# eric-zqwang/puzzlefusion-plusplus

Hardware: AMD Instinct MI355X
Metric: denoiser DDPM-step throughput (fragment*steps/s) (higher is better)
Workload: dtype f32 (GEMMs: f16x3); 1 GPU; DDPM training iteration, BASELINE configs[1]: add_noise + rotate + frozen PointNet++/VQ encode (in the loop) + DenoiserTransformer forward (dropouts on) + MSE + full backward + [encoder of iteration i+1 issued on its own stream during iteration i] AdamW; padded_slots=not evaluated (their gradient contribution is exactly zero), puzzles_per_gpu=32, fragment_slots=20, points_per_fragment=1024, valid_fragments_per_gpu=154, weights=random init, reference architecture (57.6M denoiser + 0.6M encoder params)

## Files before the change

### include/pfpp.h

```cpp
#ifndef PFPP_H_
#define PFPP_H_

#include <stddef.h>
#include <stdint.h>

#ifdef __cplusplus
extern "C" {
#endif

#define PFPP_OK 0
#define PFPP_EINVAL (-1)
#define PFPP_EUNSUPPORTED (-2)
#define PFPP_EHIP (-3)

typedef void* pfpp_stream_t;

#define PFPP_ABI_VERSION 2
int pfpp_version(void);
const char* pfpp_build_info(void);
const char* pfpp_last_error(void);
int64_t pfpp_abi_sizeof(const char* name);
int pfpp_device_cu_count(void);
int pfpp_set_attention_mode(int mode);
int pfpp_get_attention_mode(void);
// ... 491 lines not shown
int pfpp_gemm_wd_f16(const pfpp_planes* A, int64_t lda, const pfpp_pw* w, const float* bias, const float* residual, int64_t ldr, float* out,
                     int64_t ldc, int64_t M, int64_t N, int64_t K, pfpp_stream_t stream);
#define PFPP_REBLOCK_MAX 32
typedef struct pfpp_reblock_job { pfpp_planes w; int64_t N, K, ldw; void *fhi, *flo; int32_t transposed; } pfpp_reblock_job;
int pfpp_reblock_planes(const pfpp_reblock_job* jobs, int32_t n, pfpp_stream_t stream);
int pfpp_layernorm_linear_small(const float* x, const float* mod, int64_t ld_mod, const float* gamma, const float* beta,
                                const int32_t* group_batch, int64_t group_rows, const pfpp_pw* w, const float* bias, float* out,
                                int64_t ldc, const pfpp_planes* u_planes, int64_t ldu, int64_t M, int64_t N, int64_t C, float eps,
                                pfpp_stream_t stream);

typedef struct pfpp_head_params {
  pfpp_planes w0, w2;
  const float *w4, *b0, *b2, *b4;
  pfpp_planes f0, f2;
} pfpp_head_params;
typedef struct pfpp_head_grads { float *w4, *b4, *b2, *b0; } pfpp_head_grads;
int pfpp_heads_fwd(const float* pooled, const pfpp_head_params* trans, const pfpp_head_params* rot, int64_t R, int64_t C,
                   float* a0, float* v0, float* a1, float* v1, float* out, const int32_t* slot, int64_t ldo,
                   pfpp_stream_t stream);
int pfpp_heads_bwd(const float* dout, const int32_t* slot, const pfpp_head_params* trans, const pfpp_head_params* rot, int64_t R, int64_t C,
                   const float* a0, const float* v0, const float* a1, const float* v1, float* da0, float* da1, float* dp,
                   const pfpp_head_grads* g_trans, const pfpp_head_grads* g_rot, float grad_scale, float* dx, int64_t L,
                   pfpp_stream_t stream);

int pfpp_verifier_attn_fwd(const float* qkv, float* out, float* lse, const uint8_t* key_valid, int64_t B, int64_t E, int64_t H,
                           int64_t dh, float scale, float p, uint64_t seed, uint32_t site, pfpp_stream_t stream);
int pfpp_verifier_attn_bwd(const float* qkv, const float* out, const float* dout, const float* lse, float* dqkv,
                           const uint8_t* key_valid, int64_t B, int64_t E, int64_t H, int64_t dh, float scale, float p, uint64_t seed,
                           uint32_t site, pfpp_stream_t stream);
int pfpp_verifier_attn_dropout_mask(uint8_t* keep, int64_t B, int64_t H, int64_t E, float p, uint64_t seed, uint32_t site,
                                    pfpp_stream_t stream);

int pfpp_verifier_head_bce(const float* h6, const float* w, const float* b, const float* target, const uint8_t* valid,
                           const float* dlogit_in, int64_t M, int64_t C, float neg_weight, float* logits, float* dlogit, float* dh6, float* dw, float* db, float* loss,
                           int32_t* stats, float* amax, double* workspace, pfpp_stream_t stream);
int64_t pfpp_verifier_head_bce_workspace(void);

int pfpp_verifier_gelu_dropout(const float* z, float* u, int64_t n, float p, uint64_t seed, uint32_t site, pfpp_stream_t stream);
int pfpp_verifier_gelu_dropout_bwd(const float* z, const float* du, float* dz, int64_t n, float p, uint64_t seed, uint32_t site,
                                   pfpp_stream_t stream);

int pfpp_chamfer_fwd(const float* off, const float* ctr, int64_t rep, const float* tgt, float* d_src, int32_t* i_src,
                     float* d_tgt, int32_t* i_tgt, int64_t batch, int64_t n, int64_t m, pfpp_stream_t stream);
int pfpp_chamfer_bwd(const float* off, const float* ctr, int64_t rep, const float* tgt, const int32_t* i_src, const int32_t* i_tgt,
                     float* grad, int64_t batch, int64_t n, int64_t m, float scale, const float* gscale, pfpp_stream_t stream);
int pfpp_chamfer_reduce(const float* d_src, int64_t n_src, const float* d_tgt, int64_t n_tgt, float scale, float* loss,
// ... 65 lines not shown
```

### puzzlefusion-plusplus_amd/csrc/heads.hip

```cpp
#include "pfpp_common.h"

namespace {

typedef _Float16 half8 __attribute__((ext_vector_type(8)));
typedef _Float16 half4 __attribute__((ext_vector_type(4)));
typedef float f32x16 __attribute__((ext_vector_type(16)));

constexpr int HC = 512;
constexpr int HC2 = 256;
constexpr int KP = HC + 8;
constexpr int NW = 8;

__device__ __forceinline__ float silu_f(float v) { return v / (1.0f + expf(-v)); }
__device__ __forceinline__ float silu_grad(float v) {
  const float s = 1.0f / (1.0f + expf(-v));
  return s * (1.0f + v * (1.0f - s));
}

struct HeadW {
  const _Float16 *w0h, *w0l, *w2h, *w2l;
  const half8 *f0h, *f0l, *f2h, *f2l;
  const float *w4, *b0, *b2, *b4;
  float inv_s0, inv_s2;
  int n_out, c0;
// ... 64 lines not shown
  const int S = K / 16, NG = K / 64;
  half8 bh[2][4][NT], bl[2][4][NT];
  auto fetch = [&](int g, int slot) {
#pragma unroll
    for (int j = 0; j < NT; ++j)
#pragma unroll
      for (int u = 0; u < 4; ++u) {
        const size_t blk = (size_t)(tile0 + j) * S + 4 * g + u;
        bh[slot][u][j] = fh[blk * 64 + lane];
        bl[slot][u][j] = fl[blk * 64 + lane];
      }
  };
  fetch(0, 0);
  for (int g = 0; g < NG; g += 2) {
#pragma unroll
    for (int half = 0; half < 2; ++half) {
      const int gg = g + half;
      if (gg < NG) {
        fetch(gg + 1 < NG ? gg + 1 : NG - 1, half ^ 1);
        __builtin_amdgcn_sched_barrier(0);
#pragma unroll
        for (int u = 0; u < 4; ++u) {
          const half8 a_h = ah[2 * (4 * gg + u)], a_l = al[2 * (4 * gg + u)];
#pragma unroll
          for (int j = 0; j < NT; ++j) {
            acc[j] = __builtin_amdgcn_mfma_f32_32x32x16_f16(a_l, bh[half][u][j], acc[j], 0, 0, 0);
            acc[j] = __builtin_amdgcn_mfma_f32_32x32x16_f16(a_h, bl[half][u][j], acc[j], 0, 0, 0);
            acc[j] = __builtin_amdgcn_mfma_f32_32x32x16_f16(a_h, bh[half][u][j], acc[j], 0, 0, 0);
          }
        }
        __builtin_amdgcn_sched_barrier(0);
      }
    }
  }
}

__device__ __forceinline__ void zero(f32x16& a) {
#pragma unroll
  for (int e = 0; e < 16; ++e) a[e] = 0.0f;
}

__global__ __launch_bounds__(64 * NW) void heads_fwd_kernel(HeadsFwdP p) {
  extern __shared__ __align__(16) char hd_smem[];
  _Float16* sh = reinterpret_cast<_Float16*>(hd_smem);
  _Float16* sl = sh + 32 * KP;
  const int tid = threadIdx.x, lane = tid & 63, wave = tid >> 6, l31 = lane & 31, lhi = lane >> 5;
// ... 48 lines not shown
#pragma unroll
    for (int e = 0; e < 16; ++e) {
      const int row = (e & 3) + 8 * (e >> 2) + 4 * lhi;
      const float a = acc[0][e] * w.inv_s2 + b;
      const float v = silu_f(a);
      if (p.a1 && r0 + row < R) {
        p.a1[((size_t)hd * R + r0 + row) * HC2 + col] = a;
        p.v1[((size_t)hd * R + r0 + row) * HC2 + col] = v;
      }
      sv[row * (HC2 + 1) + col] = v;
    }
    __syncthreads();
    if (tid < 32 * 4) {
      const int row = tid >> 2, c = tid & 3;
      if (c < w.n_out && r0 + row < R) {
        const float* wr = w.w4 + (size_t)c * HC2;
        float s = 0.0f;
#pragma unroll 8
        for (int k = 0; k < HC2; ++k) s = fmaf(sv[row * (HC2 + 1) + k], wr[k], s);
        const int64_t orow = p.slot ? p.slot[r0 + row] : (r0 + row);
        p.out[orow * p.ldo + w.c0 + c] = s + w.b4[c];
      }
    }
  }
}

struct HeadsBwdP {
  const float* dout;
  const int32_t* slot;
  HeadW w[2];
  const float *a0, *v0, *a1, *v1;
  float *da0, *da1;
  float* dp;
  float *gw4[2], *gb4[2], *gb2[2], *gb0[2];
  float G;
  int R;
};

__device__ __forceinline__ half4 lds_rd_tr(uint32_t addr) {
  half4 v;
  asm volatile("ds_read_b64_tr_b16 %0, %1" : "=v"(v) : "v"(addr) : "memory");
  return v;
}

__device__ __forceinline__ void contract_kmajor(const _Float16* sh, const _Float16* sl, const _Float16* __restrict__ wh,
                                                const _Float16* __restrict__ wl, int K, int ldw, int n0, _Float16* patch,
// ... 137 lines not shown
        sl[row * KP + col] = l;
      }
      cs += __shfl_xor(cs, 32);
      if (lhi == 0) unsafeAtomicAdd(p.gb0[hd] + col, cs);
    }
    __syncthreads();
  }
  {
    f32x16 acc[2];
    zero(acc[0]); zero(acc[1]);
    contract_kmajor(sh, sl, w.w0h, w.w0l, HC, HC, 64 * wave, patch, acc);
#pragma unroll
    for (int j = 0; j < 2; ++j) {
      const int col = 64 * wave + 32 * j + l31;
#pragma unroll
      for (int e = 0; e < 16; ++e) {
        const int row = (e & 3) + 8 * (e >> 2) + 4 * lhi;
        if (r0 + row < R) p.dp[((size_t)hd * R + r0 + row) * HC + col] = acc[j][e] * (invG * w.inv_s0);
      }
    }
  }
}

__global__ __launch_bounds__(256) void pool_bwd2_kernel(const float* __restrict__ dp0, const float* __restrict__ dp1, float* __restrict__ dx,
                                                        int64_t n, int L, int C) {
  const int64_t i4 = ((int64_t)blockIdx.x * 256 + threadIdx.x) * 4;
  if (i4 >= n * L * C) return;
  const int64_t row = i4 / C;
  const int c = (int)(i4 - row * C);
  const int64_t f = row / L;
  const float4 a = *reinterpret_cast<const float4*>(dp0 + f * C + c);
  const float4 b = *reinterpret_cast<const float4*>(dp1 + f * C + c);
  const float inv = 1.0f / (float)L;
  float4 v;
  v.x = (a.x + b.x) * inv; v.y = (a.y + b.y) * inv; v.z = (a.z + b.z) * inv; v.w = (a.w + b.w) * inv;
  *reinterpret_cast<float4*>(dx + i4) = v;
}

bool fill_head(HeadW& w, const pfpp_head_params& h, int n_out, int c0) {
  if (!(h.w0.hi && h.w0.lo && h.w2.hi && h.w2.lo && h.w4 && h.b0 && h.b2 && h.b4)) return false;
  w.w0h = (const _Float16*)h.w0.hi; w.w0l = (const _Float16*)h.w0.lo;
  w.w2h = (const _Float16*)h.w2.hi; w.w2l = (const _Float16*)h.w2.lo;
  const bool frag = h.f0.hi && h.f0.lo && h.f2.hi && h.f2.lo;
  w.f0h = frag ? (const half8*)h.f0.hi : nullptr; w.f0l = frag ? (const half8*)h.f0.lo : nullptr;
  w.f2h = frag ? (const half8*)h.f2.hi : nullptr; w.f2l = frag ? (const half8*)h.f2.lo : nullptr;
  w.w4 = h.w4; w.b0 = h.b0; w.b2 = h.b2; w.b4 = h.b4;
  w.inv_s0 = 1.0f / h.w0.scale; w.inv_s2 = 1.0f / h.w2.scale;
  w.n_out = n_out; w.c0 = c0;
  return true;
}

}

extern "C" int pfpp_heads_fwd(const float* pooled, const pfpp_head_params* trans, const pfpp_head_params* rot, int64_t R, int64_t C,
                              float* a0, float* v0, float* a1, float* v1, float* out, const int32_t* slot, int64_t ldo,
                              pfpp_stream_t stream) {
  PFPP_REQUIRE(pooled && trans && rot && out, "null pointer");
  PFPP_SUPPORTED(C == HC, "width != 512");
  PFPP_REQUIRE((!a0 && !v0 && !a1 && !v1) || (a0 && v0 && a1 && v1), "the saved activations come all or none");
  PFPP_REQUIRE(ldo >= 7 && pfpp::aligned16(pooled), "ldo < 7 or misaligned input");
  if (R == 0) return PFPP_OK;
  HeadsFwdP p;
  PFPP_REQUIRE(fill_head(p.w[0], *trans, 3, 0) && fill_head(p.w[1], *rot, 4, 3), "null weight pointer");
  p.x = pooled; p.a0 = a0; p.v0 = v0; p.a1 = a1; p.v1 = v1; p.out = out; p.slot = slot; p.ldo = (int)ldo; p.R = (int)R;
  const size_t smem = (size_t)2 * 32 * KP * sizeof(_Float16);
  if (pfpp_allow_dyn_lds<heads_fwd_kernel>((int)smem) != hipSuccess) return pfpp::check_launch(__func__);
  hipLaunchKernelGGL(heads_fwd_kernel, dim3((unsigned)((R + 31) / 32), 2), dim3(64 * NW), smem, pfpp::as_stream(stream), p);
  return pfpp::check_launch(__func__);
}

extern "C" int pfpp_heads_bwd(const float* dout, const int32_t* slot, const pfpp_head_params* trans, const pfpp_head_params* rot, int64_t R, int64_t C,
                              const float* a0, const float* v0, const float* a1, const float* v1, float* da0, float* da1, float* dp,
                              const pfpp_head_grads* g_trans, const pfpp_head_grads* g_rot, float grad_scale, float* dx, int64_t L,
                              pfpp_stream_t stream) {
  PFPP_REQUIRE(dout && trans && rot && a0 && v0 && a1 && v1 && da0 && da1 && dp && g_trans && g_rot, "null pointer");
  PFPP_SUPPORTED(C == HC, "width != 512");
  PFPP_REQUIRE(grad_scale > 0.0f && L >= 1, "bad grad_scale / L");
  if (R == 0) return PFPP_OK;
  HeadsBwdP p;
  PFPP_REQUIRE(fill_head(p.w[0], *trans, 3, 0) && fill_head(p.w[1], *rot, 4, 3), "null weight pointer");
  const pfpp_head_grads* gs[2] = {g_trans, g_rot};
  for (int h = 0; h < 2; ++h) {
    PFPP_REQUIRE(gs[h]->w4 && gs[h]->b4 && gs[h]->b2 && gs[h]->b0, "null gradient pointer");
    p.gw4[h] = gs[h]->w4; p.gb4[h] = gs[h]->b4; p.gb2[h] = gs[h]->b2; p.gb0[h] = gs[h]->b0;
  }
  p.dout = dout; p.slot = slot; p.a0 = a0; p.v0 = v0; p.a1 = a1; p.v1 = v1; p.da0 = da0; p.da1 = da1; p.dp = dp; p.G = grad_scale; p.R = (int)R;
  hipStream_t st = pfpp::as_stream(stream);
  const size_t smem = (size_t)2 * 32 * KP * sizeof(_Float16) + (size_t)NW * 8192;
  if (pfpp_allow_dyn_lds<heads_bwd_kernel>((int)smem) != hipSuccess) return pfpp::check_launch(__func__);
  hipLaunchKernelGGL(heads_bwd_kernel, dim3((unsigned)((R + 31) / 32), 2), dim3(64 * NW), smem, st, p);
  if (dx) {
    const int64_t total = R * L * C;
    hipLaunchKernelGGL(pool_bwd2_kernel, dim3((unsigned)((total / 4 + 255) / 256)), dim3(256), 0, st, dp, dp + R * C, dx, R, (int)L, (int)C);
  }
  return pfpp::check_launch(__func__);
}
```

### puzzlefusion-plusplus_amd/pfpp_hip/_lib.py

```python
from __future__ import annotations

import ctypes as C
import os
from pathlib import Path

LIB_PATH = Path(os.environ["PFPP_LIB_PATH"]).resolve() if os.environ.get("PFPP_LIB_PATH") else Path(__file__).resolve().parent / "libpfpp_hip.so"

_p = C.c_void_p
_i64 = C.c_int64
_i32 = C.c_int32
_f32 = C.c_float


class GemmArgs(C.Structure):

    _fields_ = [
        ("A", _p), ("W", _p), ("C", _p),
        ("w_hi", _p), ("w_lo", _p),
        ("a_hi", _p), ("a_lo", _p), ("c_hi", _p), ("c_lo", _p),
        ("bias", _p), ("scale", _p), ("shift", _p), ("residual", _p),
        ("M", _i64), ("N", _i64), ("K", _i64),
        ("lda", _i64), ("ldw", _i64), ("ldc", _i64), ("ldr", _i64),
        ("w_kmajor", _i32), ("act", _i32), ("pool", _i32),
        ("batch", _i32), ("zdiv", _i32), ("precision", _i32),
# ... 141 lines not shown

class DwJob(C.Structure):

    _fields_ = [("dy", PlanesC), ("x", PlanesC), ("gw", _p), ("gb", _p), ("M", _i64), ("N", _i64)]


class ReblockJob(C.Structure):

    _fields_ = [("w", PlanesC), ("N", _i64), ("K", _i64), ("ldw", _i64), ("fhi", _p), ("flo", _p), ("transposed", _i32)]


SIGNATURES = {
    "pfpp_tlayers_eval": [C.POINTER(TlayersEvalArgs), _p],
    "pfpp_embed_tokens_small": [_p, _p, _p, _p, _p, C.POINTER(PwC), _p, _p, _p, _p, _p, _p, _i64, _i64, _i64, _p],
    "pfpp_gemm_small": [_pl, _i64, C.POINTER(PwC), _p, _p, _i64, _p, _i64, _i64, _i64, _i64, _p],
    "pfpp_gemm_wd": [_pl, _i64, C.POINTER(PwC), _p, _p, _i64, _p, _i64, _i64, _i64, _i64, _p],
    "pfpp_gemm_wd_supported": [_i64, _i64, _i64],
    "pfpp_gemm_wd_f16": [_pl, _i64, C.POINTER(PwC), _p, _p, _i64, _p, _i64, _i64, _i64, _i64, _p],
    "pfpp_reblock_planes": [C.POINTER(ReblockJob), _i32, _p],
    "pfpp_layernorm_linear_small": [_p, _p, _i64, _p, _p, _p, _i64, C.POINTER(PwC), _p, _p, _i64, _pl, _i64, _i64, _i64, _i64, _f32, _p],
    "pfpp_heads_fwd": [_p, C.POINTER(HeadParams), C.POINTER(HeadParams), _i64, _i64, _p, _p, _p, _p, _p, _p, _i64, _p],
    "pfpp_heads_bwd": [_p, _p, C.POINTER(HeadParams), C.POINTER(HeadParams), _i64, _i64, _p, _p, _p, _p, _p, _p, _p,
                       C.POINTER(HeadGrads), C.POINTER(HeadGrads), _f32, _p, _i64, _p],
    "pfpp_tlayers_fwd": [C.POINTER(TlayersArgs), _i32, _i32, _p],
    "pfpp_tlayers_bwd": [C.POINTER(TlayersArgs), _i32, _i32, _p, _p],
    "pfpp_set_attention_mode": [C.c_int],
    "pfpp_se3_rotate_gather": [_p, _p, _p, _p, _i64, _i64, _p],
    "pfpp_pose_apply": [_p, _p, _p, _p, _i64, _i64, C.c_int, _p],
    "pfpp_fps": [_p, _p, _p, _i64, _i64, _i64, _p],
    "pfpp_ball_query": [_p, _p, _p, _i64, _i64, _i64, _i64, _f32, _p],
    "pfpp_sample_levels": [_p, _i64, _i64, C.POINTER(SampleLevel), _p],
    "pfpp_group_gather": [_p, _p, _p, _p, _p, _i64, _i64, _i64, _i64, _i64, _i64, _p],
    "pfpp_gemm": [C.POINTER(GemmArgs), _p],
    "pfpp_sa_mlp3_fused": [_p] * 16 + [_i64] * 7 + [_p],
    "pfpp_sa_mlp2_fused": [_p] * 13 + [_i64] * 7 + [_p],
    "pfpp_sa_mlp2_fused_p": [_p] * 13 + [_pl] + [_i64] * 7 + [_p],
    "pfpp_sa_mlp2_table_p": [_p] * 11 + [_pl] + [_i64] * 8 + [_p],
    "pfpp_sa_table_planes": [_p] * 7 + [_pl] + [_i64] * 6 + [_p],
    "pfpp_vq_encode": [_p, _p, _p, _p, _p, _i64, _i64, _i64, _i64, _p],
    "pfpp_scatter_rows": [_p, _p, _p, _i64, _i64, _p],
    "pfpp_token_features": [_p, _p, _p, _p, _p, _p, _i64, _i64, _p],
    "pfpp_token_features_slots": [_p, _p, _p, _p, _p, _p, _p, _i64, _i64, _p],
    "pfpp_token_combine_slots": [_p, _p, _p, _p, _p, _p, _p, _p, _i64, _i64, _i64, _p],
    "pfpp_token_combine_bwd_slots": [_p, _p, _p, _p, _p, _i64, _i64, _i64, _p],
    "pfpp_mse_loss_masked": [_p, _p, _p, _p, _p, _p, _p, _i64, _i64, _f32, _p],
    "pfpp_token_combine": [_p, _p, _p, _p, _p, _p, _i64, _i64, _i64, _i64, _p],
# ... 89 lines not shown
    "pfpp_mesh_status": [_p, _p],
    "pfpp_match_classify_compact": [_p, _p, _p, _p, _f32, _p, _p, _i64, _i64, _p, _p, _p, _p, _p],
    "pfpp_match_gather_rows": [_p, _p, _p, _p, _p, _p, _p, _i64, _i64, _i64, _p, _p, _p],
    "pfpp_match_normalize_halves": [_p, _i64, _i64, _p],
    "pfpp_sinkhorn_masked": [_p, _i64, _p, _i64, _f32, _i64, _p, _p, _p, _p, _i64, _p],
    "pfpp_fracture_labels": [_p, _p, _p, _p, _i64, _i64, _p, _p, _p],
    "pfpp_ragged_fps": [_p, _p, _p, _i64, _i64, _i64, _p, _p, _p],
    "pfpp_ragged_knn": [_p, _p, _p, _p, _i64, _i64, _i64, _i64, _p, _p, _p],
    "pfpp_ragged_group": [_p, _i64, _i64, _p, _p, _p, _i64, _i64, _i64, _i64, _p, _i64, _p],
    "pfpp_ragged_interp": [_p, _p, _p, _p, _p, _i64, _p, _i64, _i64, _i64, _p, _i64, _p, _p],
    "pfpp_feat_knn": [_p, _i64, _p, _i64, _i64, _i64, _i64, _i64, _p, _p],
    "pfpp_ptf_aggregate": [_p, _p, _p, _i64, _p, _p, _p, _p, _i64, _i64, _i64, _p, _p],
    "pfpp_attn_rows16": [_p, _p, _p, _p, _i64, _i64, _i64, _i64, _f32, _p],
    "pfpp_layernorm128": [_p, _p, _p, _p, _i64, _i64, _f32, _p],
}
PLAIN = {
    "pfpp_version": ([], C.c_int),
    "pfpp_last_error": ([], C.c_char_p),
    "pfpp_build_info": ([], C.c_char_p),
    "pfpp_abi_sizeof": ([C.c_char_p], C.c_int64),
    "pfpp_last_gemm_kernel": ([], C.c_char_p),
    "pfpp_device_cu_count": ([], C.c_int),
    "pfpp_get_attention_mode": ([], C.c_int),
    "pfpp_ada_linear_bwd_scratch_floats": ([_i64, _i64], C.c_int64),
    "pfpp_token_features_t_cols": ([_i64, _i64], C.c_int64),
    "pfpp_tlayers_fwd_bytes": ([_i64, _i64, _i64, _i64], C.c_int64),
    "pfpp_tlayers_frag_bytes": ([_i64, _i64], C.c_int64),
    "pfpp_tlayers_fwd_hout_offset": ([_i64, _i64, _i64, _i64], C.c_int64),
    "pfpp_tlayers_bwd_bytes": ([_i64, _i64, _i64, _i64], C.c_int64),
    "pfpp_bn_stats_workspace": ([_i64, _i64], C.c_int64),
    "pfpp_fragment_prepare_workspace": ([_i64, _i64], C.c_int64),
    "pfpp_verifier_head_bce_workspace": ([], C.c_int64),
    "pfpp_vq_train_workspace": ([_i64, _i64], C.c_int64),
    "pfpp_bn_relu_bwd_workspace": ([_i64, _i64], C.c_int64),
    "pfpp_mesh_vertex_graph_workspace": ([_p, _i64, _p], C.c_int64),
    "pfpp_sinkhorn_workspace": ([_i64], C.c_int64),
}

STRUCT_MIRRORS = {
    "sample_level": SampleLevel, "gemm_args": GemmArgs, "planes": PlanesC, "slab_job": SlabJob, "gemm_planes_args": GemmPlanesArgs,
    "sa_train_args": SaTrainArgs, "gemm_grad_args": GemmGradArgs, "tlayer_params": TlayerParams, "tlayer_grads": TlayerGrads,
    "tlayer_adamw": TlayerAdamw, "tlayers_args": TlayersArgs, "pw": PwC, "elayer_params": ElayerParams,
    "tlayers_eval_args": TlayersEvalArgs, "head_params": HeadParams, "head_grads": HeadGrads, "reblock_job": ReblockJob, "dw_job": DwJob,
}

ACT = {"none": 0, "relu": 1, "silu": 2, "gelu": 3, "geglu": 4}
# ... 75 lines not shown
```

### puzzlefusion-plusplus_amd/pfpp_hip/train_ops.py

```python
from __future__ import annotations

import ctypes as C
from typing import Optional, Tuple

import torch

from . import _lib
from ._lib import ACT, GemmGradArgs, check
from . import ops
from .ops import _chk, _ptr, _stream

_f32 = torch.float32
import os as _os

SPLIT_DX = _os.environ.get("PFPP_SPLIT_DX", "1") == "1"


def gemm_grad(A: torch.Tensor, W: torch.Tensor, out: torch.Tensor, *, M: int, N: int, K: int, lda: int, ldw: int,
              ldc: int, a_kmajor: bool = False, w_kmajor: bool = False, accumulate: bool = False,
              split_k: int = 0, batch: int = 1, sA: int = 0, sW: int = 0, sC: int = 0, a_scale: float = 1.0,
              w_scale: float = 1.0, alpha: float = 1.0, a_off: int = 0, w_off: int = 0, c_off: int = 0,
              colsum: Optional[torch.Tensor] = None) -> torch.Tensor:
    _chk(A, _f32, "A"); _chk(W, _f32, "W"); _chk(out, _f32, "out")
    a = GemmGradArgs()
# ... 617 lines not shown
def attn_blockdiag_bwd_planes(qkv, dout, n_frag: int, L: int, H: int, dh: int, scale: float, g_scale: float):
    from .planes import Planes, _pl

    _chk(qkv, _f32, "qkv"); _chk(dout, _f32, "dout")
    dq = Planes.empty(qkv.shape[0], qkv.shape[1], qkv.device, g_scale)
    check(_lib.load().pfpp_attn_blockdiag_bwd_p(_ptr(qkv), _ptr(dout), None, n_frag, L, H, dh, scale, _pl(dq), _stream()),
          "pfpp_attn_blockdiag_bwd_p")
    return dq


def head_params(w0, w2, w4: torch.Tensor, b0: torch.Tensor, b2: torch.Tensor, b4: torch.Tensor, static: bool = False):
    from ._lib import HeadParams, PlanesC

    for t_, nm in ((w4, "w4"), (b0, "b0"), (b2, "b2"), (b4, "b4")):
        _chk(t_, _f32, nm)
    f0 = f2 = PlanesC(None, None, 0.0)
    if static:
        (h0, l0), (h2, l2) = w0.frag(), w2.frag()
        f0, f2 = PlanesC(h0.data_ptr(), l0.data_ptr(), w0.scale), PlanesC(h2.data_ptr(), l2.data_ptr(), w2.scale)
    return HeadParams(PlanesC(w0.hi.data_ptr(), w0.lo.data_ptr(), w0.scale), PlanesC(w2.hi.data_ptr(), w2.lo.data_ptr(), w2.scale),
                      w4.data_ptr(), b0.data_ptr(), b2.data_ptr(), b4.data_ptr(), f0, f2)


def heads_fwd(pooled: torch.Tensor, trans, rot, out: torch.Tensor, slot: Optional[torch.Tensor] = None, save: bool = False):
    _chk(pooled, _f32, "pooled"); _chk(out, _f32, "out")
    R, Cc = pooled.shape
    saved = (None, None, None, None)
    if save:
        saved = tuple(torch.empty((2, R, n), dtype=_f32, device=pooled.device) for n in (Cc, Cc, Cc // 2, Cc // 2))
    if slot is not None:
        _chk(slot, torch.int32, "slot")
    check(_lib.load().pfpp_heads_fwd(_ptr(pooled), C.byref(trans), C.byref(rot), R, Cc, *(_ptr(t_) for t_ in saved), _ptr(out),
                                     _ptr(slot), out.shape[-1], _stream()), "pfpp_heads_fwd")
    return saved if save else None


def heads_bwd(dout: torch.Tensor, trans, rot, saved, g_trans, g_rot, g_scale: float, L: int, want_dx: bool = True,
              slot: Optional[torch.Tensor] = None):
    _chk(dout, _f32, "dout")
    if slot is not None:
        _chk(slot, torch.int32, "slot")
    a0, v0, a1, v1 = saved
    _, R, Cc = a0.shape
    dev = dout.device
    da0 = torch.empty((2, R, Cc), dtype=_f32, device=dev)
    da1 = torch.empty((2, R, Cc // 2), dtype=_f32, device=dev)
    dp = torch.empty((2, R, Cc), dtype=_f32, device=dev)
    dx = torch.empty((R * L, Cc), dtype=_f32, device=dev) if want_dx else None
    check(_lib.load().pfpp_heads_bwd(_ptr(dout), _ptr(slot), C.byref(trans), C.byref(rot), R, Cc, _ptr(a0), _ptr(v0), _ptr(a1), _ptr(v1), _ptr(da0),
                                     _ptr(da1), _ptr(dp), C.byref(g_trans), C.byref(g_rot), g_scale, _ptr(dx), L, _stream()),
          "pfpp_heads_bwd")
    return da0, da1, (dx if want_dx else dp)


def verifier_attn_fwd(qkv: torch.Tensor, key_valid: torch.Tensor, B: int, E: int, H: int, dh: int, scale: float, p: float,
                      seed: int, site: int, out: Optional[torch.Tensor] = None) -> Tuple[torch.Tensor, torch.Tensor]:
    _chk(qkv, _f32, "qkv"); _chk(key_valid, torch.uint8, "key_valid")
    if qkv.shape != (B * E, 3 * H * dh) or key_valid.numel() != B * E:
        raise ValueError("verifier_attn_fwd: qkv must be [B*E, 3*H*dh] and key_valid [B, E]")
    if out is None:
        out = torch.empty((B * E, H * dh), dtype=_f32, device=qkv.device)
    lse = torch.empty((B * E, H), dtype=_f32, device=qkv.device)
    check(_lib.load().pfpp_verifier_attn_fwd(_ptr(qkv), _ptr(out), _ptr(lse), _ptr(key_valid), B, E, H, dh, scale, p, seed, site,
                                             _stream()), "pfpp_verifier_attn_fwd")
    return out, lse


def verifier_attn_bwd(qkv: torch.Tensor, out_fwd: torch.Tensor, dout: torch.Tensor, lse: torch.Tensor, key_valid: torch.Tensor,
                      B: int, E: int, H: int, dh: int, scale: float, p: float, seed: int, site: int,
                      out: Optional[torch.Tensor] = None) -> torch.Tensor:
    _chk(qkv, _f32, "qkv"); _chk(out_fwd, _f32, "out_fwd"); _chk(dout, _f32, "dout"); _chk(lse, _f32, "lse")
    _chk(key_valid, torch.uint8, "key_valid")
    if qkv.shape != (B * E, 3 * H * dh) or dout.shape != (B * E, H * dh) or out_fwd.shape != dout.shape or lse.shape != (B * E, H):
        raise ValueError("verifier_attn_bwd: shape mismatch")
# ... 69 lines not shown
```

Baseline: 26540 fragment*steps/s.

## Split output-head MLP forward and backward into per-layer column-sliced kernels

Replaces the single fused heads kernel (one 512-thread block per 32-row tile per head) with a sequence of per-layer launches whose grid is also sliced over output columns. The work then spreads over many more workgroups when R is small, for example about 154 rows giving only 5 tiles per head. The backward pass is split into a layer-1 kernel and a layer-0 kernel, and the layer-1 kernel carries extra blocks that compute the w4/b4/b2 gradients column-wise with atomics. The cost is more launches, activations written to and reread from global memory (a scratch buffer when nothing is saved), and more atomic traffic. An automatic selection by row count turns the new path on for R of 32 or more.

```diff
diff --git a/include/pfpp.h b/include/pfpp.h
--- a/include/pfpp.h
+++ b/include/pfpp.h
@@ -537,6 +537,15 @@
                    const float* a0, const float* v0, const float* a1, const float* v1, float* da0, float* da1, float* dp,
                    const pfpp_head_grads* g_trans, const pfpp_head_grads* g_rot, float grad_scale, float* dx, int64_t L,
                    pfpp_stream_t stream);
+int pfpp_heads_sliced_min_rows(void);
+int pfpp_last_heads_path(void);
+int pfpp_heads_fwd_path(const float* pooled, const pfpp_head_params* trans, const pfpp_head_params* rot, int64_t R, int64_t C,
+                        float* a0, float* v0, float* a1, float* v1, float* out, const int32_t* slot, int64_t ldo, int32_t path,
+                        pfpp_stream_t stream);
+int pfpp_heads_bwd_path(const float* dout, const int32_t* slot, const pfpp_head_params* trans, const pfpp_head_params* rot, int64_t R, int64_t C,
+                        const float* a0, const float* v0, const float* a1, const float* v1, float* da0, float* da1, float* dp,
+                        const pfpp_head_grads* g_trans, const pfpp_head_grads* g_rot, float grad_scale, float* dx, int64_t L,
+                        int32_t path, pfpp_stream_t stream);
 
 int pfpp_verifier_attn_fwd(const float* qkv, float* out, float* lse, const uint8_t* key_valid, int64_t B, int64_t E, int64_t H,
                            int64_t dh, float scale, float p, uint64_t seed, uint32_t site, pfpp_stream_t stream);
diff --git a/puzzlefusion-plusplus_amd/csrc/heads.hip b/puzzlefusion-plusplus_amd/csrc/heads.hip
--- a/puzzlefusion-plusplus_amd/csrc/heads.hip
+++ b/puzzlefusion-plusplus_amd/csrc/heads.hip
@@ -110,6 +110,48 @@
 #pragma unroll
         for (int u = 0; u < 4; ++u) {
           const half8 a_h = ah[2 * (4 * gg + u)], a_l = al[2 * (4 * gg + u)];
+#pragma unroll
+          for (int j = 0; j < NT; ++j) {
+            acc[j] = __builtin_amdgcn_mfma_f32_32x32x16_f16(a_l, bh[half][u][j], acc[j], 0, 0, 0);
+            acc[j] = __builtin_amdgcn_mfma_f32_32x32x16_f16(a_h, bl[half][u][j], acc[j], 0, 0, 0);
+            acc[j] = __builtin_amdgcn_mfma_f32_32x32x16_f16(a_h, bh[half][u][j], acc[j], 0, 0, 0);
+          }
+        }
+        __builtin_amdgcn_sched_barrier(0);
+      }
+    }
+  }
+}
+
+template <int NT>
+__device__ __forceinline__ void contract_frag_rm(const _Float16* sh, const _Float16* sl, const half8* __restrict__ fh, const half8* __restrict__ fl,
+                                                 int K, int tile0, f32x16 (&acc)[NT]) {
+  const int lane = threadIdx.x & 63, l31 = lane & 31, lhi = lane >> 5;
+  const half8* ah = reinterpret_cast<const half8*>(sh + l31 * KP + 32 * lhi);
+  const half8* al = reinterpret_cast<const half8*>(sl + l31 * KP + 32 * lhi);
+  const int S = K / 16, NG = K / 64;
+  half8 bh[2][4][NT], bl[2][4][NT];
+  auto fetch = [&](int g, int slot) {
+#pragma unroll
+    for (int j = 0; j < NT; ++j)
+#pragma unroll
+      for (int u = 0; u < 4; ++u) {
+        const size_t blk = (size_t)(tile0 + j) * S + 4 * g + 2 * lhi + (u >> 1);
+        bh[slot][u][j] = fh[blk * 64 + 32 * (u & 1) + l31];
+        bl[slot][u][j] = fl[blk * 64 + 32 * (u & 1) + l31];
+      }
+  };
+  fetch(0, 0);
+  for (int g = 0; g < NG; g += 2) {
+#pragma unroll
+    for (int half = 0; half < 2; ++half) {
+      const int gg = g + half;
+      if (gg < NG) {
+        fetch(gg + 1 < NG ? gg + 1 : NG - 1, half ^ 1);
+        __builtin_amdgcn_sched_barrier(0);
+#pragma unroll
+        for (int u = 0; u < 4; ++u) {
+          const half8 a_h = ah[8 * gg + u], a_l = al[8 * gg + u];
 #pragma unroll
           for (int j = 0; j < NT; ++j) {
             acc[j] = __builtin_amdgcn_mfma_f32_32x32x16_f16(a_l, bh[half][u][j], acc[j], 0, 0, 0);
@@ -204,6 +246,108 @@
         p.out[orow * p.ldo + w.c0 + c] = s + w.b4[c];
       }
     }
+  }
+}
+
+constexpr int SL_W0 = 4;
+constexpr int SL_W1 = 2;
+
+template <int THREADS>
+__device__ __forceinline__ void stage_rows(const float* __restrict__ src, int r0, int R, float g, _Float16* sh, _Float16* sl) {
+  constexpr int N = 32 * HC / 4 / THREADS, U = 16;
+  static_assert(N % U == 0, "stage_rows: whole batches");
+  for (int b = 0; b < N; b += U) {
+    float4 v[U];
+#pragma unroll
+    for (int u = 0; u < U; ++u) {
+      const int i = threadIdx.x + (b + u) * THREADS, row = i / (HC / 4), c = (i - row * (HC / 4)) * 4;
+      v[u] = make_float4(0.f, 0.f, 0.f, 0.f);
+      if (r0 + row < R) v[u] = *reinterpret_cast<const float4*>(src + (size_t)(r0 + row) * HC + c);
+    }
+#pragma unroll
+    for (int u = 0; u < U; ++u) {
+      const int i = threadIdx.x + (b + u) * THREADS, row = i / (HC / 4), c = (i - row * (HC / 4)) * 4;
+      half4 h, l;
+      PFPP_SPLIT_TO(v[u].x * g, h[0], l[0]); PFPP_SPLIT_TO(v[u].y * g, h[1], l[1]); PFPP_SPLIT_TO(v[u].z * g, h[2], l[2]);
+      PFPP_SPLIT_TO(v[u].w * g, h[3], l[3]);
+      *reinterpret_cast<half4*>(sh + row * KP + c) = h;
+      *reinterpret_cast<half4*>(sl + row * KP + c) = l;
+    }
+  }
+}
+
+template <int LAYER, int WAVES>
+__global__ __launch_bounds__(64 * WAVES) void heads_fwd_layer_kernel(HeadsFwdP p) {
+  extern __shared__ __align__(16) char hd_smem[];
+  _Float16* sh = reinterpret_cast<_Float16*>(hd_smem);
+  _Float16* sl = sh + 32 * KP;
+  const int tid = threadIdx.x, lane = tid & 63, wave = tid >> 6, l31 = lane & 31, lhi = lane >> 5;
+  const int hd = blockIdx.z, r0 = blockIdx.x * 32, R = p.R;
+  const int n0 = (blockIdx.y * WAVES + wave) * 32;
+  constexpr int NOUT = LAYER == 0 ? HC : HC2;
+  const HeadW w = p.w[hd];
+  stage_rows<64 * WAVES>(LAYER == 0 ? p.x : p.v0 + (size_t)hd * R * HC, r0, R, 1.0f, sh, sl);
+  __syncthreads();
+  f32x16 acc[1];
+  zero(acc[0]);
+  const half8* fh = LAYER == 0 ? w.f0h : w.f2h;
+  const half8* fl = LAYER == 0 ? w.f0l : w.f2l;
+  if (fh) contract_frag_rm<1>(sh, sl, fh, fl, HC, n0 / 32, acc);
+  else contract_rowmajor<1>(sh, sl, LAYER == 0 ? w.w0h : w.w2h, LAYER == 0 ? w.w0l : w.w2l, HC, HC, n0, acc);
+  const int col = n0 + l31;
+  const float b = (LAYER == 0 ? w.b0 : w.b2)[col];
+  const float inv_s = LAYER == 0 ? w.inv_s0 : w.inv_s2;
+  float* pa = LAYER == 0 ? p.a0 : p.a1;
+  float* pv = LAYER == 0 ? p.v0 : p.v1;
+#pragma unroll
+  for (int e = 0; e < 16; ++e) {
+    const int row = (e & 3) + 8 * (e >> 2) + 4 * lhi;
+    const float a = acc[0][e] * inv_s + b;
+    const float v = silu_f(a);
+    if (r0 + row < R) {
+      if (pa) pa[((size_t)hd * R + r0 + row) * NOUT + col] = a;
+      pv[((size_t)hd * R + r0 + row) * NOUT + col] = v;
+    }
+  }
+}
+
+constexpr int LAST_ROWS = 8;
+__global__ __launch_bounds__(64) void heads_fwd_last_kernel(HeadsFwdP p) {
+  __shared__ float sv[LAST_ROWS * (HC2 + 1)];
+  __shared__ float sw[4 * (HC2 + 1)];
+  const int tid = threadIdx.x;
+  const int hd = blockIdx.y, r0 = blockIdx.x * LAST_ROWS, R = p.R;
+  const HeadW w = p.w[hd];
+  float4 v[LAST_ROWS * HC2 / 4 / 64];
+  float u[4][4];
+#pragma unroll
+  for (int q = 0; q < LAST_ROWS * HC2 / 4 / 64; ++q) {
+    const int i = tid + 64 * q, row = i / (HC2 / 4), c = (i - row * (HC2 / 4)) * 4;
+    v[q] = make_float4(0.f, 0.f, 0.f, 0.f);
+    if (r0 + row < R) v[q] = *reinterpret_cast<const float4*>(p.v1 + ((size_t)hd * R + r0 + row) * HC2 + c);
+  }
+#pragma unroll
+  for (int q = 0; q < 4; ++q)
+#pragma unroll
+    for (int i = 0; i < 4; ++i) u[q][i] = q < w.n_out ? w.w4[(size_t)q * HC2 + tid + 64 * i] : 0.0f;
+#pragma unroll
+  for (int q = 0; q < LAST_ROWS * HC2 / 4 / 64; ++q) {
+    const int i = tid + 64 * q, row = i / (HC2 / 4), c = (i - row * (HC2 / 4)) * 4;
+    float* d = sv + row * (HC2 + 1) + c;
+    d[0] = v[q].x; d[1] = v[q].y; d[2] = v[q].z; d[3] = v[q].w;
+  }
+#pragma unroll
+  for (int q = 0; q < 4; ++q)
+#pragma unroll
+    for (int i = 0; i < 4; ++i) sw[q * (HC2 + 1) + tid + 64 * i] = u[q][i];
+  __syncthreads();
+  const int row = tid >> 2, c = tid & 3;
+  if (row < LAST_ROWS && c < w.n_out && r0 + row < R) {
+    float s = 0.0f;
+#pragma unroll 16
+    for (int k = 0; k < HC2; ++k) s = fmaf(sv[row * (HC2 + 1) + k], sw[c * (HC2 + 1) + k], s);
+    const int64_t orow = p.slot ? p.slot[r0 + row] : (r0 + row);
+    p.out[orow * p.ldo + w.c0 + c] = s + w.b4[c];
   }
 }
 
@@ -387,6 +531,150 @@
   }
 }
 
+constexpr int SL_WB = 2;
+
+constexpr int BWD_SLICES = HC / (64 * SL_WB);
+
+__device__ __forceinline__ void a1_column(const HeadsBwdP& p, int hd, int r0, int k, float (&a)[32]) {
+  const int R = p.R;
+#pragma unroll
+  for (int r = 0; r < 32; ++r) a[r] = r0 + r < R ? p.a1[((size_t)hd * R + r0 + r) * HC2 + k] : 0.0f;
+}
+__device__ __forceinline__ void da1_column(const HeadW& w, const float (*s_do)[4], int r0, int R, int k, const float (&a)[32], float (&d)[32]) {
+  float wk[4];
+#pragma unroll
+  for (int c = 0; c < 4; ++c) wk[c] = c < w.n_out ? w.w4[(size_t)c * HC2 + k] : 0.0f;
+#pragma unroll
+  for (int r = 0; r < 32; ++r) {
+    d[r] = 0.0f;
+    if (r0 + r < R) {
+      float dv = 0.0f;
+#pragma unroll
+      for (int c = 0; c < 4; ++c) dv = fmaf(s_do[r][c], wk[c], dv);
+      d[r] = dv * silu_grad(a[r]);
+    }
+  }
+}
+
+__global__ __launch_bounds__(64 * SL_WB) void heads_bwd_l1_kernel(HeadsBwdP p) {
+  extern __shared__ __align__(16) char hd_smem[];
+  _Float16* sh = reinterpret_cast<_Float16*>(hd_smem);
+  _Float16* sl = sh + 32 * KP;
+  _Float16* patches = sl + 32 * KP;
+  __shared__ float s_do[32][4];
+  const int tid = threadIdx.x, lane = tid & 63, wave = tid >> 6, l31 = lane & 31, lhi = lane >> 5;
+  const int hd = blockIdx.z, r0 = blockIdx.x * 32, R = p.R;
+  const HeadW w = p.w[hd];
+  const float G = p.G, invG = 1.0f / G;
+  {
+    const int row = tid >> 2, c = tid & 3;
+    s_do[row][c] = (c < w.n_out && r0 + row < R) ? p.dout[(size_t)(p.slot ? p.slot[r0 + row] : r0 + row) * 7 + w.c0 + c] : 0.0f;
+  }
+  if (blockIdx.y >= BWD_SLICES) {
+    const int k = (blockIdx.y - BWD_SLICES) * (64 * SL_WB) + tid;
+    float v[32], a[32], d[32], s[4] = {0.0f, 0.0f, 0.0f, 0.0f};
+#pragma unroll
+    for (int r = 0; r < 32; ++r) v[r] = r0 + r < R ? p.v1[((size_t)hd * R + r0 + r) * HC2 + k] : 0.0f;
+    a1_column(p, hd, r0, k, a);
+    __syncthreads();
+    if (blockIdx.y == BWD_SLICES && tid < 4) {
+      float sb = 0.0f;
+      for (int r = 0; r < 32; ++r) sb += s_do[r][tid];
+      if (tid < w.n_out) unsafeAtomicAdd(p.gb4[hd] + tid, sb);
+    }
+#pragma unroll
+    for (int r = 0; r < 32; ++r)
+      if (r0 + r < R) {
+#pragma unroll
+        for (int c = 0; c < 4; ++c) s[c] = fmaf(s_do[r][c], v[r], s[c]);
+      }
+#pragma unroll
+    for (int c = 0; c < 4; ++c)
+      if (c < w.n_out) unsafeAtomicAdd(p.gw4[hd] + (size_t)c * HC2 + k, s[c]);
+    da1_column(w, s_do, r0, R, k, a, d);
+    float cs = 0.0f;
+#pragma unroll
+    for (int r = 0; r < 32; ++r) {
+      if (r0 + r < R) p.da1[((size_t)hd * R + r0 + r) * HC2 + k] = d[r];
+      cs += d[r];
+    }
+    unsafeAtomicAdd(p.gb2[hd] + k, cs);
+    return;
+  }
+  const int n0 = (blockIdx.y * SL_WB + wave) * 64;
+  float a1v[HC2 / (64 * SL_WB)][32], a0v[2][16];
+#pragma unroll
+  for (int q = 0; q < HC2 / (64 * SL_WB); ++q) a1_column(p, hd, r0, tid + q * 64 * SL_WB, a1v[q]);
+#pragma unroll
+  for (int j = 0; j < 2; ++j)
+#pragma unroll
+    for (int e = 0; e < 16; ++e) {
+      const int row = (e & 3) + 8 * (e >> 2) + 4 * lhi;
+      a0v[j][e] = r0 + row < R ? p.a0[((size_t)hd * R + r0 + row) * HC + n0 + 32 * j + l31] : 0.0f;
+    }
+  __syncthreads();
+#pragma unroll
+  for (int q = 0; q < HC2 / (64 * SL_WB); ++q) {
+    const int k = tid + q * 64 * SL_WB;
+    float d[32];
+    da1_column(w, s_do, r0, R, k, a1v[q], d);
+#pragma unroll
+    for (int r = 0; r < 32; ++r) {
+      _Float16 h, l;
+      PFPP_SPLIT_TO(d[r] * G, h, l);
+      sh[r * KP + k] = h;
+      sl[r * KP + k] = l;
+    }
+  }
+  __syncthreads();
+  f32x16 acc[2];
+  zero(acc[0]); zero(acc[1]);
+  contract_kmajor(sh, sl, w.w2h, w.w2l, HC2, HC, n0, patches + wave * 4096, acc);
+#pragma unroll
+  for (int j = 0; j < 2; ++j) {
+    const int col = n0 + 32 * j + l31;
+    float cs = 0.0f;
+#pragma unroll
+    for (int e = 0; e < 16; ++e) {
+      const int row = (e & 3) + 8 * (e >> 2) + 4 * lhi;
+      float d = 0.0f;
+      if (r0 + row < R) {
+        d = acc[j][e] * (invG * w.inv_s2) * silu_grad(a0v[j][e]);
+        p.da0[((size_t)hd * R + r0 + row) * HC + col] = d;
+      }
+      cs += d;
+    }
+    cs += __shfl_xor(cs, 32);
+    if (lhi == 0) unsafeAtomicAdd(p.gb0[hd] + col, cs);
+  }
+}
+
+__global__ __launch_bounds__(64 * SL_WB) void heads_bwd_l0_kernel(HeadsBwdP p) {
+  extern __shared__ __align__(16) char hd_smem[];
+  _Float16* sh = reinterpret_cast<_Float16*>(hd_smem);
+  _Float16* sl = sh + 32 * KP;
+  _Float16* patches = sl + 32 * KP;
+  const int tid = threadIdx.x, lane = tid & 63, wave = tid >> 6, l31 = lane & 31, lhi = lane >> 5;
+  const int hd = blockIdx.z, r0 = blockIdx.x * 32, R = p.R;
+  const HeadW w = p.w[hd];
+  const float invG = 1.0f / p.G;
+  stage_rows<64 * SL_WB>(p.da0 + (size_t)hd * R * HC, r0, R, p.G, sh, sl);
+  __syncthreads();
+  f32x16 acc[2];
+  zero(acc[0]); zero(acc[1]);
+  const int n0 = (blockIdx.y * SL_WB + wave) * 64;
+  contract_kmajor(sh, sl, w.w0h, w.w0l, HC, HC, n0, patches + wave * 4096, acc);
+#pragma unroll
+  for (int j = 0; j < 2; ++j) {
+    const int col = n0 + 32 * j + l31;
+#pragma unroll
+    for (int e = 0; e < 16; ++e) {
+      const int row = (e & 3) + 8 * (e >> 2) + 4 * lhi;
+      if (r0 + row < R) p.dp[((size_t)hd * R + r0 + row) * HC + col] = acc[j][e] * (invG * w.inv_s0);
+    }
+  }
+}
+
 __global__ __launch_bounds__(256) void pool_bwd2_kernel(const float* __restrict__ dp0, const float* __restrict__ dp1, float* __restrict__ dx,
                                                         int64_t n, int L, int C) {
   const int64_t i4 = ((int64_t)blockIdx.x * 256 + threadIdx.x) * 4;
@@ -415,32 +703,66 @@
   return true;
 }
 
-}
-
-extern "C" int pfpp_heads_fwd(const float* pooled, const pfpp_head_params* trans, const pfpp_head_params* rot, int64_t R, int64_t C,
-                              float* a0, float* v0, float* a1, float* v1, float* out, const int32_t* slot, int64_t ldo,
-                              pfpp_stream_t stream) {
+constexpr int64_t HEADS_SLICED_MIN_ROWS = 32;
+enum { HEADS_AUTO = 0, HEADS_SINGLE = 1, HEADS_SLICED = 2 };
+std::atomic<int> g_last_heads_path{0};
+
+}
+
+extern "C" int pfpp_heads_sliced_min_rows(void) { return (int)HEADS_SLICED_MIN_ROWS; }
+extern "C" int pfpp_last_heads_path(void) { return g_last_heads_path.load(std::memory_order_relaxed); }
+
+extern "C" int pfpp_heads_fwd_path(const float* pooled, const pfpp_head_params* trans, const pfpp_head_params* rot, int64_t R, int64_t C,
+                                   float* a0, float* v0, float* a1, float* v1, float* out, const int32_t* slot, int64_t ldo,
+                                   int32_t path, pfpp_stream_t stream) {
   PFPP_REQUIRE(pooled && trans && rot && out, "null pointer");
   PFPP_SUPPORTED(C == HC, "width != 512");
   PFPP_REQUIRE((!a0 && !v0 && !a1 && !v1) || (a0 && v0 && a1 && v1), "the saved activations come all or none");
   PFPP_REQUIRE(ldo >= 7 && pfpp::aligned16(pooled), "ldo < 7 or misaligned input");
+  PFPP_REQUIRE(path == HEADS_AUTO || path == HEADS_SINGLE || path == HEADS_SLICED, "path is not 0 (by R), 1 (single launch) or 2 (sliced)");
+  PFPP_REQUIRE(path != HEADS_SLICED || (v0 && pfpp::aligned16(v0) && pfpp::aligned16(v1)),
+               "the sliced path needs the activation buffers (16-byte aligned)");
+  PFPP_REQUIRE(R >= 0 && R <= (int64_t)65535 * 32, "bad row count");
   if (R == 0) return PFPP_OK;
   HeadsFwdP p;
   PFPP_REQUIRE(fill_head(p.w[0], *trans, 3, 0) && fill_head(p.w[1], *rot, 4, 3), "null weight pointer");
   p.x = pooled; p.a0 = a0; p.v0 = v0; p.a1 = a1; p.v1 = v1; p.out = out; p.slot = slot; p.ldo = (int)ldo; p.R = (int)R;
   const size_t smem = (size_t)2 * 32 * KP * sizeof(_Float16);
+  const unsigned tiles = (unsigned)((R + 31) / 32);
+  hipStream_t st = pfpp::as_stream(stream);
+  const bool sliced = path == HEADS_SLICED ||
+                      (path == HEADS_AUTO && R >= HEADS_SLICED_MIN_ROWS && v0 && pfpp::aligned16(v0) && pfpp::aligned16(v1));
+  g_last_heads_path.store(sliced ? HEADS_SLICED : HEADS_SINGLE, std::memory_order_relaxed);
+  if (sliced) {
+    if (pfpp_allow_dyn_lds<heads_fwd_layer_kernel<0, SL_W0>>((int)smem) != hipSuccess ||
+        pfpp_allow_dyn_lds<heads_fwd_layer_kernel<1, SL_W1>>((int)smem) != hipSuccess)
+      return pfpp::check_launch(__func__);
+    hipLaunchKernelGGL((heads_fwd_layer_kernel<0, SL_W0>), dim3(tiles, HC / (32 * SL_W0), 2), dim3(64 * SL_W0), smem, st, p);
+    hipLaunchKernelGGL((heads_fwd_layer_kernel<1, SL_W1>), dim3(tiles, HC2 / (32 * SL_W1), 2), dim3(64 * SL_W1), smem, st, p);
+    hipLaunchKernelGGL(heads_fwd_last_kernel, dim3((unsigned)((R + LAST_ROWS - 1) / LAST_ROWS), 2), dim3(64), 0, st, p);
+    return pfpp::check_launch(__func__);
+  }
   if (pfpp_allow_dyn_lds<heads_fwd_kernel>((int)smem) != hipSuccess) return pfpp::check_launch(__func__);
-  hipLaunchKernelGGL(heads_fwd_kernel, dim3((unsigned)((R + 31) / 32), 2), dim3(64 * NW), smem, pfpp::as_stream(stream), p);
+  hipLaunchKernelGGL(heads_fwd_kernel, dim3(tiles, 2), dim3(64 * NW), smem, st, p);
   return pfpp::check_launch(__func__);
 }
 
-extern "C" int pfpp_heads_bwd(const float* dout, const int32_t* slot, const pfpp_head_params* trans, const pfpp_head_params* rot, int64_t R, int64_t C,
-                              const float* a0, const float* v0, const float* a1, const float* v1, float* da0, float* da1, float* dp,
-                              const pfpp_head_grads* g_trans, const pfpp_head_grads* g_rot, float grad_scale, float* dx, int64_t L,
+extern "C" int pfpp_heads_fwd(const float* pooled, const pfpp_head_params* trans, const pfpp_head_params* rot, int64_t R, int64_t C,
+                              float* a0, float* v0, float* a1, float* v1, float* out, const int32_t* slot, int64_t ldo,
                               pfpp_stream_t stream) {
+  return pfpp_heads_fwd_path(pooled, trans, rot, R, C, a0, v0, a1, v1, out, slot, ldo, HEADS_AUTO, stream);
+}
+
+extern "C" int pfpp_heads_bwd_path(const float* dout, const int32_t* slot, const pfpp_head_params* trans, const pfpp_head_params* rot, int64_t R,
+                                   int64_t C, const float* a0, const float* v0, const float* a1, const float* v1, float* da0, float* da1,
+                                   float* dp, const pfpp_head_grads* g_trans, const pfpp_head_grads* g_rot, float grad_scale, float* dx,
+                                   int64_t L, int32_t path, pfpp_stream_t stream) {
   PFPP_REQUIRE(dout && trans && rot && a0 && v0 && a1 && v1 && da0 && da1 && dp && g_trans && g_rot, "null pointer");
   PFPP_SUPPORTED(C == HC, "width != 512");
   PFPP_REQUIRE(grad_scale > 0.0f && L >= 1, "bad grad_scale / L");
+  PFPP_REQUIRE(path == HEADS_AUTO || path == HEADS_SINGLE || path == HEADS_SLICED, "path is not 0 (by R), 1 (single launch) or 2 (sliced)");
+  PFPP_REQUIRE(path != HEADS_SLICED || pfpp::aligned16(da0), "the sliced path reads da0 back in 16-byte pieces: misaligned");
+  PFPP_REQUIRE(R >= 0 && R <= (int64_t)65535 * 32, "bad row count");
   if (R == 0) return PFPP_OK;
   HeadsBwdP p;
   PFPP_REQUIRE(fill_head(p.w[0], *trans, 3, 0) && fill_head(p.w[1], *rot, 4, 3), "null weight pointer");
@@ -451,12 +773,30 @@
   }
   p.dout = dout; p.slot = slot; p.a0 = a0; p.v0 = v0; p.a1 = a1; p.v1 = v1; p.da0 = da0; p.da1 = da1; p.dp = dp; p.G = grad_scale; p.R = (int)R;
   hipStream_t st = pfpp::as_stream(stream);
-  const size_t smem = (size_t)2 * 32 * KP * sizeof(_Float16) + (size_t)NW * 8192;
-  if (pfpp_allow_dyn_lds<heads_bwd_kernel>((int)smem) != hipSuccess) return pfpp::check_launch(__func__);
-  hipLaunchKernelGGL(heads_bwd_kernel, dim3((unsigned)((R + 31) / 32), 2), dim3(64 * NW), smem, st, p);
+  const unsigned tiles = (unsigned)((R + 31) / 32);
+  const bool sliced = path == HEADS_SLICED || (path == HEADS_AUTO && R >= HEADS_SLICED_MIN_ROWS && pfpp::aligned16(da0));
+  g_last_heads_path.store(sliced ? HEADS_SLICED : HEADS_SINGLE, std::memory_order_relaxed);
+  if (sliced) {
+    const size_t smem = (size_t)2 * 32 * KP * sizeof(_Float16) + (size_t)SL_WB * 8192;
+    if (pfpp_allow_dyn_lds<heads_bwd_l1_kernel>((int)smem) != hipSuccess || pfpp_allow_dyn_lds<heads_bwd_l0_kernel>((int)smem) != hipSuccess)
+      return pfpp::check_launch(__func__);
+    hipLaunchKernelGGL(heads_bwd_l1_kernel, dim3(tiles, BWD_SLICES + HC2 / (64 * SL_WB), 2), dim3(64 * SL_WB), smem, st, p);
+    hipLaunchKernelGGL(heads_bwd_l0_kernel, dim3(tiles, BWD_SLICES, 2), dim3(64 * SL_WB), smem, st, p);
+  } else {
+    const size_t smem = (size_t)2 * 32 * KP * sizeof(_Float16) + (size_t)NW * 8192;
+    if (pfpp_allow_dyn_lds<heads_bwd_kernel>((int)smem) != hipSuccess) return pfpp::check_launch(__func__);
+    hipLaunchKernelGGL(heads_bwd_kernel, dim3(tiles, 2), dim3(64 * NW), smem, st, p);
+  }
   if (dx) {
     const int64_t total = R * L * C;
     hipLaunchKernelGGL(pool_bwd2_kernel, dim3((unsigned)((total / 4 + 255) / 256)), dim3(256), 0, st, dp, dp + R * C, dx, R, (int)L, (int)C);
   }
   return pfpp::check_launch(__func__);
 }
+
+extern "C" int pfpp_heads_bwd(const float* dout, const int32_t* slot, const pfpp_head_params* trans, const pfpp_head_params* rot, int64_t R, int64_t C,
+                              const float* a0, const float* v0, const float* a1, const float* v1, float* da0, float* da1, float* dp,
+                              const pfpp_head_grads* g_trans, const pfpp_head_grads* g_rot, float grad_scale, float* dx, int64_t L,
+                              pfpp_stream_t stream) {
+  return pfpp_heads_bwd_path(dout, slot, trans, rot, R, C, a0, v0, a1, v1, da0, da1, dp, g_trans, g_rot, grad_scale, dx, L, HEADS_AUTO, stream);
+}
diff --git a/puzzlefusion-plusplus_amd/pfpp_hip/_lib.py b/puzzlefusion-plusplus_amd/pfpp_hip/_lib.py
--- a/puzzlefusion-plusplus_amd/pfpp_hip/_lib.py
+++ b/puzzlefusion-plusplus_amd/pfpp_hip/_lib.py
@@ -187,6 +187,9 @@
     "pfpp_heads_fwd": [_p, C.POINTER(HeadParams), C.POINTER(HeadParams), _i64, _i64, _p, _p, _p, _p, _p, _p, _i64, _p],
     "pfpp_heads_bwd": [_p, _p, C.POINTER(HeadParams), C.POINTER(HeadParams), _i64, _i64, _p, _p, _p, _p, _p, _p, _p,
                        C.POINTER(HeadGrads), C.POINTER(HeadGrads), _f32, _p, _i64, _p],
+    "pfpp_heads_fwd_path": [_p, C.POINTER(HeadParams), C.POINTER(HeadParams), _i64, _i64, _p, _p, _p, _p, _p, _p, _i64, _i32, _p],
+    "pfpp_heads_bwd_path": [_p, _p, C.POINTER(HeadParams), C.POINTER(HeadParams), _i64, _i64, _p, _p, _p, _p, _p, _p, _p,
+                            C.POINTER(HeadGrads), C.POINTER(HeadGrads), _f32, _p, _i64, _i32, _p],
     "pfpp_tlayers_fwd": [C.POINTER(TlayersArgs), _i32, _i32, _p],
     "pfpp_tlayers_bwd": [C.POINTER(TlayersArgs), _i32, _i32, _p, _p],
     "pfpp_set_attention_mode": [C.c_int],
@@ -322,6 +325,8 @@
     "pfpp_last_gemm_kernel": ([], C.c_char_p),
     "pfpp_device_cu_count": ([], C.c_int),
     "pfpp_get_attention_mode": ([], C.c_int),
+    "pfpp_heads_sliced_min_rows": ([], C.c_int),
+    "pfpp_last_heads_path": ([], C.c_int),
     "pfpp_ada_linear_bwd_scratch_floats": ([_i64, _i64], C.c_int64),
     "pfpp_token_features_t_cols": ([_i64, _i64], C.c_int64),
     "pfpp_tlayers_fwd_bytes": ([_i64, _i64, _i64, _i64], C.c_int64),
diff --git a/puzzlefusion-plusplus_amd/pfpp_hip/train_ops.py b/puzzlefusion-plusplus_amd/pfpp_hip/train_ops.py
--- a/puzzlefusion-plusplus_amd/pfpp_hip/train_ops.py
+++ b/puzzlefusion-plusplus_amd/pfpp_hip/train_ops.py
@@ -663,24 +663,58 @@
                       w4.data_ptr(), b0.data_ptr(), b2.data_ptr(), b4.data_ptr(), f0, f2)
 
 
-def heads_fwd(pooled: torch.Tensor, trans, rot, out: torch.Tensor, slot: Optional[torch.Tensor] = None, save: bool = False):
+HEADS_PATH = {None: 0, "single": 1, "sliced": 2}
+_heads_scratch = {}
+
+
+def heads_sliced_min_rows() -> int:
+    return _lib.load().pfpp_heads_sliced_min_rows()
+
+
+def last_heads_path() -> Optional[str]:
+    return {0: None, 1: "single", 2: "sliced"}[_lib.load().pfpp_last_heads_path()]
+
+
+def _heads_path(path) -> int:
+    if path not in HEADS_PATH:
+        raise ValueError(f"heads: path must be None, 'single' or 'sliced', not {path!r}")
+    return HEADS_PATH[path]
+
+
+def heads_fwd(pooled: torch.Tensor, trans, rot, out: torch.Tensor, slot: Optional[torch.Tensor] = None, save: bool = False,
+              path: Optional[str] = None):
+    code = _heads_path(path)
     _chk(pooled, _f32, "pooled"); _chk(out, _f32, "out")
     R, Cc = pooled.shape
     saved = (None, None, None, None)
     if save:
         saved = tuple(torch.empty((2, R, n), dtype=_f32, device=pooled.device) for n in (Cc, Cc, Cc // 2, Cc // 2))
+    elif R > 0 and (code == 2 or (code == 0 and R >= heads_sliced_min_rows())):
+        need = 2 * R * 3 * Cc
+        key = (pooled.device, torch.cuda.current_stream(pooled.device).cuda_stream)
+        if torch.cuda.is_current_stream_capturing():
+            buf = torch.empty(need, dtype=_f32, device=pooled.device)
+        else:
+            buf = _heads_scratch.get(key)
+            if buf is None or buf.numel() < need:
+                buf = _heads_scratch[key] = torch.empty(need, dtype=_f32, device=pooled.device)
+        o, saved = 0, []
+        for n in (Cc, Cc, Cc // 2, Cc // 2):
+            saved.append(buf[o:o + 2 * R * n].view(2, R, n))
+            o += 2 * R * n
     if slot is not None:
         _chk(slot, torch.int32, "slot")
-    check(_lib.load().pfpp_heads_fwd(_ptr(pooled), C.byref(trans), C.byref(rot), R, Cc, *(_ptr(t_) for t_ in saved), _ptr(out),
-                                     _ptr(slot), out.shape[-1], _stream()), "pfpp_heads_fwd")
-    return saved if save else None
+    check(_lib.load().pfpp_heads_fwd_path(_ptr(pooled), C.byref(trans), C.byref(rot), R, Cc, *(_ptr(t_) for t_ in saved), _ptr(out),
+                                          _ptr(slot), out.shape[-1], code, _stream()), "pfpp_heads_fwd")
+    return tuple(saved) if save else None
 
 
 def heads_bwd(dout: torch.Tensor, trans, rot, saved, g_trans, g_rot, g_scale: float, L: int, want_dx: bool = True,
-              slot: Optional[torch.Tensor] = None):
+              slot: Optional[torch.Tensor] = None, path: Optional[str] = None):
     _chk(dout, _f32, "dout")
     if slot is not None:
         _chk(slot, torch.int32, "slot")
+    code = _heads_path(path)
     a0, v0, a1, v1 = saved
     _, R, Cc = a0.shape
     dev = dout.device
@@ -688,9 +722,9 @@
     da1 = torch.empty((2, R, Cc // 2), dtype=_f32, device=dev)
     dp = torch.empty((2, R, Cc), dtype=_f32, device=dev)
     dx = torch.empty((R * L, Cc), dtype=_f32, device=dev) if want_dx else None
-    check(_lib.load().pfpp_heads_bwd(_ptr(dout), _ptr(slot), C.byref(trans), C.byref(rot), R, Cc, _ptr(a0), _ptr(v0), _ptr(a1), _ptr(v1), _ptr(da0),
-                                     _ptr(da1), _ptr(dp), C.byref(g_trans), C.byref(g_rot), g_scale, _ptr(dx), L, _stream()),
-          "pfpp_heads_bwd")
+    check(_lib.load().pfpp_heads_bwd_path(_ptr(dout), _ptr(slot), C.byref(trans), C.byref(rot), R, Cc, _ptr(a0), _ptr(v0), _ptr(a1), _ptr(v1),
+                                          _ptr(da0), _ptr(da1), _ptr(dp), C.byref(g_trans), C.byref(g_rot), g_scale, _ptr(dx), L, code,
+                                          _stream()), "pfpp_heads_bwd")
     return da0, da1, (dx if want_dx else dp)
 
 
```

Result: no change. 26670 fragment*steps/s (median of 6 runs) (+0.5%).
